# openzklib/openzl

Measured on AMD Instinct MI355X. Metric: MSM points/sec (BLS12-381 G1), higher is better.
Workload: dtype u32; 1 GPU; bls12_381_g1_msm_2^24_per_gpu; points_per_gpu=16777216, curve=BLS12-381 G1, scalars=uniform < r (255 bit), window_bits=20, windows=13, precomputed_table=none (the fixed-key table mode is reported separately as msm_fixed_key), parallelism=single

## Files before the change

### openzl_amd/csrc/zl_msm.hip

```cpp
#include <stdlib.h>
#include <string.h>
#include <stdio.h>
#include <algorithm>
#include <chrono>
#include <condition_variable>
#include <mutex>
#include <thread>
#include <vector>
#include "zl_ctx.h"
#include "zl_pool.h"
#include "zl_quad.h"

#ifndef ZL_G
#error "compile with -DZL_G=<group config>"
#endif
#include "zl_msm_job.h"
#include "zl_msm_bases.h"
ZL_MSM_ACCUMULATE_KERNELS(extern, ZL_G)
ZL_MSM_TAIL_KERNELS(extern, ZL_G)

template <class G>
static int msm_run_t(zl_ctx* ctx, const zl_bases& bs, size_t first, const void* d_scalars, size_t n, uint64_t* out_partial) {
    using X = XYZZ<typename G::F>;
    X total = X::inf();
// ... 67 lines not shown
    for (size_t i = 0; i < count; i++) any_empty = any_empty || specs[i].n == 0;
    if (any_empty || count == 1) {
        for (size_t i = 0; i < count; i++) {
            if (recorded) { while (recorded->load(std::memory_order_acquire) >= 0 && recorded->load(std::memory_order_acquire) <= (int)i) std::this_thread::yield(); if (recorded->load() < 0) return ZL_EHIP; }
            if (specs[i].wait) ZL_HIP(ctx, hipEventSynchronize(specs[i].wait));
            int rc = msm_run_t<G>(ctx, *specs[i].bs, specs[i].first, specs[i].d_scalars, specs[i].n, out_partials + i * ZL_PARTIAL_WORDS);
            if (rc) return rc;
            if (on_done) (*on_done)(i);
        }
        return ZL_OK;
    }
    int rc;
    struct Busy {
        std::atomic<int>& f;
        bool mine;
        explicit Busy(std::atomic<int>& x) : f(x), mine(x.exchange(1, std::memory_order_acq_rel) == 0) {}
        ~Busy() { if (mine) f.store(0, std::memory_order_release); }
    } busy(ctx->pipeline_busy);
    if (!busy.mine) return ZL_EINVAL;
    if (!ctx->stream_sort) {
        int prio_lo = 0, prio_hi = 0;
        (void)hipDeviceGetStreamPriorityRange(&prio_lo, &prio_hi);
        ZL_HIP(ctx, hipStreamCreateWithPriority(&ctx->stream_sort, hipStreamNonBlocking, prio_hi));
        for (auto& t : ctx->stream_tail) ZL_HIP(ctx, hipStreamCreateWithPriority(&t, hipStreamNonBlocking, prio_hi));
    }
    std::vector<MsmJob<G>> jobs(count);
    size_t t5 = 0, t6 = 0;
    uint32_t max_sets = 0;
    bool one_key = true;
    for (size_t i = 1; i < count; i++) one_key = one_key && specs[i].bs == specs[0].bs && specs[i].first == specs[0].first && specs[i].n == specs[0].n;
    uint64_t biggest = 0;
    for (size_t i = 0; i < count; i++) biggest = std::max<uint64_t>(biggest, (uint64_t)specs[i].n);
    const bool side = biggest <= ((uint64_t)1 << zl_tune("ZL_TUNE_SIDE_BY_SIDE_LOG", 20));
    const size_t NS = side ? std::min<size_t>(count, (size_t)std::min(4, std::max(1, zl_tune("ZL_TUNE_SIDE_LANES", 4)))) : 3;
    for (size_t i = 0; i < count; i++) {
        if ((rc = jobs[i].plan(ctx, *specs[i].bs, specs[i].first, specs[i].d_scalars, specs[i].n, (one_key && !side) ? 18 : MsmJob<G>::phi_slot_of((int)(i % NS))))) return rc;
        if (one_key && !side && i > 0) jobs[i].phi_owner = false;
        size_t a5, a6;
        jobs[i].sort_tmp_sizes(a5, a6);
        t5 = std::max(t5, a5);
        t6 = std::max(t6, a6);
        max_sets = std::max<uint32_t>(max_sets, jobs[i].SETS * jobs[i].roots_per_set);
    }
    hipStream_t* const lanes = ctx->stream_lane;
    if (side) {
        for (size_t k = 0; k < 4; k++)
            if (!lanes[k]) ZL_HIP(ctx, hipStreamCreateWithFlags(&lanes[k], hipStreamNonBlocking));
    }
    void* dummy;
    if (!side && t5 && (rc = zl_scratch_get(ctx, 5, t5, &dummy))) return rc;
    if (!side && t6 && (rc = zl_scratch_get(ctx, 6, t6, &dummy))) return rc;
    for (int pass = 0; pass < 2; pass++) {
        for (size_t i = 0; i < count; i++) {
            if ((rc = jobs[i].alloc(ctx, (int)(i % NS), side))) return rc;
            if (one_key && !side && i > 0 && jobs[i].glv && !jobs[i].phi_cached) jobs[i].d_phi = jobs[0].d_phi;
        }
    }
    const size_t per = sizeof(X) * (max_sets + 1) + 16;
    if (ctx->pinned_cap < per * count) {
        const size_t want = std::max(per * count, (sizeof(X) * 320 + 16) * (size_t)24);
        if (ctx->pinned) (void)hipHostFree(ctx->pinned);
        ctx->pinned = nullptr;
        ctx->pinned_cap = 0;
        ZL_HIP(ctx, hipHostMalloc(&ctx->pinned, want, hipHostMallocDefault));
        ctx->pinned_cap = want;
    }
    for (size_t i = 0; i < count; i++) {
        unsigned char* base = reinterpret_cast<unsigned char*>(ctx->pinned) + per * i;
        jobs[i].set_host_buffer(reinterpret_cast<X*>(base));
    }
// ... 450 lines not shown
```

### openzl_amd/csrc/zl_msm_job.h

```cpp
#pragma once
#include <chrono>
#include <stdlib.h>
#include <string.h>
#include <stdio.h>
#include <algorithm>
#include <vector>
#include "zl_ctx.h"
#include "zl_pool.h"
#include "zl_msm_sort.h"
#include "zl_msm_endo.h"
#include "zl_msm_accumulate.h"
#include "zl_msm_reduce.h"

static int zl_pick_window(size_t n, int sc_bits, bool wide16 = false ) {
    const double per_bucket = (double)zl_tune("ZL_TUNE_BUCKET_COST_X10", sc_bits > 200 ? 45 : 52) / 10.0;
    double best = 1e300;
    int best_c = 2;
    for (int c = 2; c <= 20; c++) {
        int W = (sc_bits + 1 + c - 1) / c;
        if (c > 16 && (((uint64_t)W << (c - 1)) >> 15) > 255) continue;
        const bool lds_sort = c < 16 || (c == 16 && !wide16);
        double cost = (double)n * W * (lds_sort ? 1.10 : 1.0) + per_bucket * W * (double)(1u << (c - 1));
        if (cost < best) { best = cost; best_c = c; }
    }
// ... 9 lines not shown
}
static int zl_pick_window_quarter(size_t n_points) {
    if (n_points < 2) return 0;
    int lg = 63 - __builtin_clzll((unsigned long long)n_points);
    if ((double)n_points >= 1.4142 * (double)((size_t)1 << lg)) lg++;
    static const signed char best[9] = {9, 0, 11, 12, 13, 13, 13, 13, 14};
    return lg >= 10 && lg <= 18 ? best[lg - 10] : 0;
}

static int zl_pick_window_precomp(size_t n, int sc_bits) {
    if (n < (size_t)700000) return 16;
    if (n < ((size_t)1 << 21)) return 20;
    double best = 1e300;
    int best_c = 16;
    for (int c = 20; c <= 23; c++) {
        int W = (sc_bits + 1 + c - 1) / c;
        double cost = (double)n * W + 6.0 * (double)(1u << (c - 1));
        if (cost < best) { best = cost; best_c = c; }
    }
    return best_c;
}

template <class G>
struct MsmJob {
    using F = typename G::F;
    using X = XYZZ<F>;
    bool pre = false;
    int c = 0, W = 0;
    int spread_t = -1;
    bool wide = false;
    bool glv = false;
    bool phi_cached = false;
    bool phi_owner = false;
    int sc_bits = 0, phi_slot = -1, endo_k = 1;
    int slotA = 5, slotB = 6;
    size_t n_real = 0;
    uint32_t* d_vs = nullptr;
    const Affine<F>* d_phi = nullptr;
    uint32_t H = 0, SETS = 0, NB = 0, ZL_CHUNK = 0, nchunks = 0, scan_blocks = 0, max_big = 0, max_giant = 0, Gn = 0, big_span = ZL_BIG_SPAN;
    uint32_t red_g0 = 0, red_lg0 = 0, red_blocks = 0, red_levels = 0;
    uint32_t roots_per_set = 0;
    uint64_t maxE = 0;
    size_t n = 0, first = 0;
    const zl_bases* bsp = nullptr;
    uint32_t *d_counts = nullptr, *d_offsets = nullptr, *d_cursor = nullptr, *d_entries = nullptr, *d_block_sums = nullptr, *d_big_list = nullptr,
             *d_big_count = nullptr, *d_ones_count = nullptr, *d_giant_count = nullptr, *d_giant_list = nullptr, *d_ones_list = nullptr,
             *d_bigsg_items = nullptr, *d_bad_scalar = nullptr;
    unsigned long long* d_bigsg_head = nullptr;
    X *d_buckets = nullptr, *d_partials = nullptr, *d_segs = nullptr, *d_stage1 = nullptr, *d_sets = nullptr, *d_ones_parts = nullptr, *d_giant_tmp = nullptr;
    const Affine<F>* d_bases = nullptr;
    const uint8_t* d_inf = nullptr;
    const uint32_t* sc = nullptr;
    X* hw = nullptr;
    uint32_t* hE = nullptr;
    std::vector<X> hw_own;
    void set_host_buffer(X* buf) {
        hw = buf;
        hE = reinterpret_cast<uint32_t*>(buf + (size_t)SETS * roots_per_set + 1);
    }

    int plan(zl_ctx* ctx, const zl_bases& bs, size_t first_, const void* d_scalars, size_t n_, int phi_slot_ = -1) {
        static const bool no_glv = getenv("ZL_NO_GLV") != nullptr;
        bool try_glv = false;
        static const size_t glv_max = (size_t)1 << zl_tune("ZL_TUNE_GLV_MAX_LOG", 19);
        if constexpr (G::GLV) try_glv = phi_slot_ >= 0 && bs.precomp_c == 0 && !no_glv && n_ >= 1 && n_ <= glv_max && (uint64_t)n_ * G::ENDO_K < (1ull << 31);
        if constexpr (G::GLV && G::ENDO_K == 2) {
// ... 212 lines not shown
        }
        const int glv_i = glv ? 1 : 0;
        (void)hipFuncSetAttribute(reinterpret_cast<const void*>(&k_msm_hist_lds), hipFuncAttributeMaxDynamicSharedMemorySize, 128 * 1024);
        (void)hipFuncSetAttribute(reinterpret_cast<const void*>(&k_msm_scatter_range), hipFuncAttributeMaxDynamicSharedMemorySize, 128 * 1024);
        if (wide) rc = sort_wide(ctx, st, sc_eff, inf_eff, bad_eff, nblk, glv_i);
        else if (c <= 16) rc = sort_lds(ctx, st, sc_eff, inf_eff, bad_eff, nblk, glv_i);
        else rc = sort_atomics(ctx, st, nblk);
        if (rc) return rc;
        ZL_HIP(ctx, hipGetLastError());
        return ZL_OK;
    }
    int sort_wide(zl_ctx* ctx, hipStream_t st, const uint32_t* sc_eff, const uint8_t* inf_eff, uint32_t* bad_eff, uint32_t nblk, int glv_i) {
        const zl_bases& bs = *bsp;
        int rc;
        uint32_t nslices = 64;
        const uint32_t max_slices = (uint32_t)((n + 4095) / 4096);
        if (nslices > max_slices) nslices = max_slices;
        const uint32_t per_slice = (uint32_t)((n + nslices - 1) / nslices);
        const uint32_t P = Gn * W * nslices;
        const uint32_t pscan_blocks = (P + SCAN_BLOCK * SCAN_ITEMS - 1) / (SCAN_BLOCK * SCAN_ITEMS);
        const size_t b_lo = (((size_t)n * W * 2 + 255) / 256) * 256, b_hi = (((size_t)n * W + 255) / 256) * 256;
        const size_t b_plo = b_lo, b_pidx = (((size_t)n * W * 4 + 255) / 256) * 256;
        const size_t b_pc = (((size_t)(2 * P + pscan_blocks + 8) * 4 + 255) / 256) * 256;
        void* pd;
        if ((rc = zl_scratch_get(ctx, slotA, b_lo + b_hi + b_plo + b_pidx + b_pc + 256, &pd))) return rc;
        unsigned char* q = (unsigned char*)pd;
        uint16_t* d_lo16 = (uint16_t*)q; q += b_lo;
        uint8_t* d_hi8 = (uint8_t*)q; q += b_hi;
        uint16_t* d_part_lo = (uint16_t*)q; q += b_plo;
        uint32_t* d_part_idx = (uint32_t*)q; q += b_pidx;
        uint32_t* d_pcounts = (uint32_t*)q;
        uint32_t* d_poff = d_pcounts + P;
        uint32_t* d_pblock = d_poff + P + 1;
        hipLaunchKernelGGL(k_msm_recode_wide, dim3(nblk), dim3(256), 0, st, sc_eff, (uint32_t)n, c, W, pre ? 0u : (H >> 15), spread_t, glv_i, d_lo16, d_hi8, d_ones_list, d_ones_count, inf_eff, sc_bits, bad_eff);
        hipLaunchKernelGGL(k_msm_part_hist, dim3(nslices, W), dim3(256), 0, st, d_hi8, (uint32_t)n, (uint32_t)W, Gn, per_slice, nslices, d_pcounts);
        hipLaunchKernelGGL(k_scan_block_sums, dim3(pscan_blocks), dim3(SCAN_BLOCK), 0, st, d_pcounts, P, d_pblock);
        hipLaunchKernelGGL(k_scan_top, dim3(1), dim3(1024), 0, st, d_pblock, pscan_blocks, d_poff + P, (const uint32_t*)nullptr);
        hipLaunchKernelGGL(k_scan_apply, dim3(pscan_blocks), dim3(SCAN_BLOCK), 0, st, d_pcounts, P, d_pblock, d_poff, d_pcounts);
        hipLaunchKernelGGL(k_msm_part_scatter_st, dim3(nslices, W), dim3(256), 0, st, d_lo16, d_hi8, (uint32_t)n, (uint32_t)W, Gn, per_slice, nslices, d_poff,
                           pre ? (uint32_t)bs.n : 0u, pre ? (uint32_t)first : 0u, d_part_lo, d_part_idx);
        const uint32_t gstride = (uint32_t)W * nslices;
        const uint32_t SG = Gn * 128;
        uint32_t fsl = 16;
        while (fsl * Gn < 2048 && fsl < 128) fsl *= 2;
        const uint32_t P2 = SG * fsl;
        const uint32_t p2scan_blocks = (P2 + SCAN_BLOCK * SCAN_ITEMS - 1) / (SCAN_BLOCK * SCAN_ITEMS);
        void* pd2;
        const size_t b2_lo = b_plo, b2_idx = b_pidx, b2_c = (((size_t)(2 * (size_t)P2 + p2scan_blocks + 8) * 4 + 255) / 256) * 256;
        if ((rc = zl_scratch_get(ctx, slotB, b2_lo + b2_idx + b2_c + 256, &pd2))) return rc;
        unsigned char* q2 = (unsigned char*)pd2;
        uint16_t* d_lo2 = (uint16_t*)q2; q2 += b2_lo;
        uint32_t* d_idx2 = (uint32_t*)q2; q2 += b2_idx;
        uint32_t* d_c2 = (uint32_t*)q2;
        uint32_t* d_off2 = d_c2 + P2;
        uint32_t* d_blk2 = d_off2 + P2 + 1;
        hipLaunchKernelGGL(k_msm_sub_hist, dim3(fsl, Gn), dim3(256), 0, st, d_part_lo, d_poff, Gn, gstride, d_poff + P, fsl, d_c2);
        hipLaunchKernelGGL(k_scan_block_sums, dim3(p2scan_blocks), dim3(SCAN_BLOCK), 0, st, d_c2, P2, d_blk2);
        hipLaunchKernelGGL(k_scan_top, dim3(1), dim3(1024), 0, st, d_blk2, p2scan_blocks, d_off2 + P2, (const uint32_t*)nullptr);
        hipLaunchKernelGGL(k_scan_apply, dim3(p2scan_blocks), dim3(SCAN_BLOCK), 0, st, d_c2, P2, d_blk2, d_off2, d_c2);
        hipLaunchKernelGGL(k_msm_sub_scatter_st, dim3(fsl, Gn), dim3(256), 0, st, d_part_lo, d_part_idx, d_poff, Gn, gstride, d_poff + P, fsl, d_off2, d_lo2,
                           d_idx2);
        hipLaunchKernelGGL(k_msm_fine_hist, dim3(SG), dim3(256), 0, st, d_lo2, d_off2, SG, fsl, d_off2 + P2, d_counts);
        hipLaunchKernelGGL(k_scan_block_sums, dim3(scan_blocks), dim3(SCAN_BLOCK), 0, st, d_counts, NB, d_block_sums);
        hipLaunchKernelGGL(k_scan_top, dim3(1), dim3(1024), 0, st, d_block_sums, scan_blocks, d_offsets + NB, (const uint32_t*)d_bad_scalar);
        hipLaunchKernelGGL(k_scan_apply, dim3(scan_blocks), dim3(SCAN_BLOCK), 0, st, d_counts, NB, d_block_sums, d_offsets, d_cursor);
        uint32_t cap = (uint32_t)std::min<uint64_t>(36 * 1024, std::max<uint64_t>(4096, (maxE / SG) * 22 / 10));
        cap = (uint32_t)std::max(1024, zl_tune("ZL_TUNE_FS_CAP", (int)cap));
        (void)hipFuncSetAttribute(reinterpret_cast<const void*>(&k_msm_fine_sort), hipFuncAttributeMaxDynamicSharedMemorySize, 160 * 1024);
        hipLaunchKernelGGL(k_msm_fine_sort, dim3(SG), dim3(zl_tune("ZL_TUNE_FS", 1024)), (size_t)(256 + cap) * 4, st, d_lo2, d_idx2, d_off2, SG, fsl, d_off2 + P2, d_offsets, cap,
                           d_entries, d_bigsg_head, d_bigsg_items);
        (void)hipFuncSetAttribute(reinterpret_cast<const void*>(&k_msm_fine_sort_big), hipFuncAttributeMaxDynamicSharedMemorySize, ZL_BT * 4);
        hipLaunchKernelGGL(k_msm_fine_sort_big, dim3(512), dim3(1024), (size_t)ZL_BT * 4, st, d_lo2, d_idx2, d_off2, SG, fsl, d_off2 + P2, d_bigsg_head,
                           d_bigsg_items, d_cursor, d_entries);
        return ZL_OK;
    }
    int sort_lds(zl_ctx* ctx, hipStream_t st, const uint32_t* sc_eff, const uint8_t* inf_eff, uint32_t* bad_eff, uint32_t nblk, int glv_i) {
        int rc;
        uint32_t nslices = (256 + W - 1) / W;
        const uint32_t max_slices = (uint32_t)((n + 4095) / 4096);
        if (nslices > max_slices) nslices = max_slices;
        if (nslices < 1) nslices = 1;
        const uint32_t per_slice = (uint32_t)((n + nslices - 1) / nslices);
        void* pd;
        if ((rc = zl_scratch_get(ctx, slotA, (size_t)n * W * 2 + (size_t)nslices * NB * 4 + 256, &pd))) return rc;
        uint16_t* d_digits = (uint16_t*)pd;
        uint32_t* d_slice_counts = (uint32_t*)((unsigned char*)pd + (((size_t)n * W * 2 + 255) / 256) * 256);
        hipLaunchKernelGGL(k_msm_recode, dim3(nblk), dim3(256), 0, st, sc_eff, (uint32_t)n, c, W, spread_t, glv_i, d_digits, d_ones_list, d_ones_count, inf_eff, sc_bits, bad_eff);
        hipLaunchKernelGGL(k_msm_hist_lds, dim3(nslices, W), dim3(1024), (size_t)H * 4, st, d_digits, (uint32_t)n, H, per_slice, NB, d_slice_counts);
        if (NB <= 14336 && nslices <= 64) {
            hipLaunchKernelGGL(k_msm_prefix_small, dim3(1), dim3(1024), ((size_t)NB + NB / 16 + 16) * 4, st, d_slice_counts, NB, nslices, d_offsets, d_cursor, (const uint32_t*)d_bad_scalar);
        } else {
        hipLaunchKernelGGL(k_msm_slice_prefix, dim3((NB + 255) / 256), dim3(256), 0, st, d_slice_counts, NB, nslices, d_counts);
        hipLaunchKernelGGL(k_scan_block_sums, dim3(scan_blocks), dim3(SCAN_BLOCK), 0, st, d_counts, NB, d_block_sums);
        hipLaunchKernelGGL(k_scan_top, dim3(1), dim3(1024), 0, st, d_block_sums, scan_blocks, d_offsets + NB, (const uint32_t*)d_bad_scalar);
        hipLaunchKernelGGL(k_scan_apply, dim3(scan_blocks), dim3(SCAN_BLOCK), 0, st, d_counts, NB, d_block_sums, d_offsets, d_cursor);
        }
        uint32_t ranges = 1;
        while (ranges * W < 256 && (H / (ranges * 2)) >= 64) ranges *= 2;
// ... 138 lines not shown
```

### openzl_amd/csrc/zl_msm_sort.h

```cpp
#pragma once
#include "zl_msm_common.h"

#define ZL_PT 4096
#define ZL_BT 16384
#define SCAN_ITEMS 16
#define SCAN_BLOCK 256

__global__ void __launch_bounds__(64) k_msm_zero_words(uint32_t* __restrict__ p, uint32_t n);
template <int MODE>
__global__ void __launch_bounds__(256) k_msm_digits(const uint32_t* __restrict__ scalars, uint32_t n, int c, int W,
                                                    uint32_t* __restrict__ counters, uint32_t* __restrict__ entries,
                                                    uint32_t* __restrict__ ones_list, uint32_t* __restrict__ ones_count, const uint8_t* __restrict__ inf,
                                                    int sc_bits, uint32_t* __restrict__ bad);
__global__ void __launch_bounds__(256) k_msm_recode(const uint32_t* __restrict__ scalars, uint32_t n, int c, int W, int spread_t, int glv, uint16_t* __restrict__ digits,
                                                             uint32_t* __restrict__ ones_list, uint32_t* __restrict__ ones_count, const uint8_t* __restrict__ inf,
                                                             int sc_bits, uint32_t* __restrict__ bad);
__global__ void __launch_bounds__(1024) k_msm_hist_lds(const uint16_t* __restrict__ digits, uint32_t n, uint32_t H, uint32_t per_slice, uint32_t NB,
                                                        uint32_t* __restrict__ counts);
__global__ void __launch_bounds__(256) k_msm_slice_prefix(uint32_t* __restrict__ counts, uint32_t NB, uint32_t nslices, uint32_t* __restrict__ tot);
__global__ void __launch_bounds__(1024) k_msm_scatter_range(const uint16_t* __restrict__ digits, uint32_t n, uint32_t H, uint32_t RB,
                                                                     const uint32_t* __restrict__ offsets, uint32_t* __restrict__ entries,
                                                                     const uint32_t* __restrict__ slice_prefix, uint32_t NB, uint32_t nslices, uint32_t per_slice,
                                                                     uint32_t parts, uint32_t W);
__global__ void __launch_bounds__(256) k_msm_recode_wide(const uint32_t* __restrict__ scalars, uint32_t n, int c, int W, uint32_t gw, int spread_t, int glv,
// ... 2 lines not shown
                                                                  int sc_bits, uint32_t* __restrict__ bad);
__global__ void __launch_bounds__(256) k_msm_part_hist(const uint8_t* __restrict__ hi8, uint32_t n, uint32_t W, uint32_t G, uint32_t per_slice,
                                                                uint32_t nslices, uint32_t* __restrict__ counts);
__global__ void __launch_bounds__(256) k_msm_sub_hist(const uint16_t* __restrict__ part_lo, const uint32_t* __restrict__ part_off, uint32_t G,
                                                               uint32_t stride, const uint32_t* __restrict__ total, uint32_t fslices,
                                                               uint32_t* __restrict__ counts);
__global__ void __launch_bounds__(256) k_msm_part_scatter_st(const uint16_t* __restrict__ lo16, const uint8_t* __restrict__ hi8, uint32_t n, uint32_t W,
                                                                      uint32_t G, uint32_t per_slice, uint32_t nslices, const uint32_t* __restrict__ part_off,
                                                                      uint32_t table_stride, uint32_t first, uint16_t* __restrict__ out_lo,
                                                                      uint32_t* __restrict__ out_idx);
__global__ void __launch_bounds__(256) k_msm_sub_scatter_st(const uint16_t* __restrict__ part_lo, const uint32_t* __restrict__ part_idx,
                                                                     const uint32_t* __restrict__ part_off, uint32_t G, uint32_t stride,
                                                                     const uint32_t* __restrict__ total, uint32_t fslices, const uint32_t* __restrict__ sub_off,
                                                                     uint16_t* __restrict__ out_lo, uint32_t* __restrict__ out_idx);
__global__ void __launch_bounds__(256) k_msm_fine_hist(const uint16_t* __restrict__ lo2, const uint32_t* __restrict__ sub_off, uint32_t SG,
                                                                uint32_t fslices, const uint32_t* __restrict__ total, uint32_t* __restrict__ counts);
__global__ void __launch_bounds__(1024) k_msm_fine_sort(const uint16_t* __restrict__ lo2, const uint32_t* __restrict__ idx2,
                                                                const uint32_t* __restrict__ sub_off, uint32_t SG, uint32_t fslices,
                                                                const uint32_t* __restrict__ total, const uint32_t* __restrict__ offsets, uint32_t cap,
                                                                uint32_t* __restrict__ entries, unsigned long long* __restrict__ big_head,
                                                                uint32_t* __restrict__ big_items);
__global__ void __launch_bounds__(1024) k_msm_fine_sort_big(const uint16_t* __restrict__ lo2, const uint32_t* __restrict__ idx2,
                                                                    const uint32_t* __restrict__ sub_off, uint32_t SG, uint32_t fslices,
                                                                    const uint32_t* __restrict__ total, const unsigned long long* __restrict__ big_head,
                                                                    const uint32_t* __restrict__ big_items, uint32_t* __restrict__ cursor,
                                                                    uint32_t* __restrict__ entries);
__global__ void __launch_bounds__(SCAN_BLOCK) k_scan_block_sums(const uint32_t* __restrict__ in, uint32_t count, uint32_t* __restrict__ block_sums);
__global__ void __launch_bounds__(1024) k_scan_top(uint32_t* __restrict__ block_sums, uint32_t nblocks, uint32_t* __restrict__ total_out,
                                                          const uint32_t* __restrict__ flag_in = nullptr );
__global__ void __launch_bounds__(1024) k_msm_prefix_small(uint32_t* __restrict__ counts, uint32_t NB, uint32_t nslices, uint32_t* __restrict__ offsets,
                                                                  uint32_t* __restrict__ cursor, const uint32_t* __restrict__ flag_in);
__global__ void __launch_bounds__(SCAN_BLOCK) k_scan_apply(const uint32_t* __restrict__ in, uint32_t count, const uint32_t* __restrict__ block_sums,
                                                           uint32_t* __restrict__ out, uint32_t* __restrict__ out2);
```

### openzl_amd/csrc/zl_msm_sort.hip

```cpp
#include "zl_msm_sort.h"



__device__ __forceinline__ bool zl_take_one(const uint32_t* s, uint32_t i, uint32_t* __restrict__ ones_list, uint32_t* __restrict__ ones_count) {
    const bool one = s[0] == 1u && (s[1] | s[2] | s[3] | s[4] | s[5] | s[6] | s[7]) == 0u;
    const uint64_t m = __ballot(one);
    if (m == 0) return false;
    const uint32_t lane = threadIdx.x & 63u;
    uint32_t base = 0;
    if (lane == (uint32_t)__ffsll((long long)m) - 1u) base = atomicAdd(ones_count, (uint32_t)__popcll(m));
    base = __shfl(base, __ffsll((long long)m) - 1);
    if (one) ones_list[base + __popcll(m & ((1ull << lane) - 1ull))] = i;
    return one;
}

__device__ __forceinline__ uint32_t zl_take_sign(uint32_t& top_word, int glv) {
    if (!glv) return 0u;
    const uint32_t sg = top_word >> 31;
    top_word &= 0x7FFFFFFFu;
    return sg;
}
__global__ void __launch_bounds__(64) k_msm_zero_words(uint32_t* __restrict__ p, uint32_t n) {
    if (threadIdx.x < n) p[threadIdx.x] = 0u;
}
// ... 188 lines not shown
    uint4 lo = sp[0], hi = sp[1];
    if (live) zl_flag_wide_scalar(hi.w, sc_bits, bad);
    if (!live || (inf && inf[i])) lo = hi = make_uint4(0, 0, 0, 0);
    uint32_t s[8] = {lo.x, lo.y, lo.z, lo.w, hi.x, hi.y, hi.z, hi.w};
    if (zl_take_one(s, i, ones_list, ones_count)) s[0] = 0;
    if (!live) return;
    const uint32_t sg = zl_take_sign(s[7], glv);
    const uint32_t H = 1u << (c - 1);
    uint32_t carry = 0;
    for (int w = 0; w < W; w++) {
        const int pos = w * c;
        const int word = pos >> 5, sh = pos & 31;
        uint64_t v = 0;
#pragma unroll
        for (int k = 0; k < 8; k++) {
            if (k == word) v |= s[k];
            if (k == word + 1) v |= (uint64_t)s[k] << 32;
        }
        uint32_t d = ((uint32_t)(v >> sh) & ((1u << c) - 1)) + carry;
        uint32_t neg = 0;
        carry = 0;
        if (d > H) { d = 2 * H - d; neg = 1; carry = 1; }
        uint32_t b = d - 1;
        if (spread_t >= 0 && w == W - 1) b |= (i & ((1u << (c - 1 - spread_t)) - 1u)) << spread_t;
        lo16[(size_t)w * n + i] = (uint16_t)((b & 0x7FFFu) | ((neg ^ sg) << 15));
        hi8[(size_t)w * n + i] = d == 0 ? (uint8_t)0xFF : (uint8_t)((uint32_t)w * gw + (b >> 15));
    }
}
__global__ void __launch_bounds__(256) k_msm_part_hist(const uint8_t* __restrict__ hi8, uint32_t n, uint32_t W, uint32_t G, uint32_t per_slice,
                                                                uint32_t nslices, uint32_t* __restrict__ counts) {
    ZL_SIDE_PRIO();
    __shared__ uint32_t hist[256];
    const uint32_t slice = blockIdx.x, w = blockIdx.y;
    hist[threadIdx.x] = 0;
    __syncthreads();
    const uint32_t lo = slice * per_slice, hi = min(n, lo + per_slice);
    const uint8_t* hw = hi8 + (size_t)w * n;
    const bool al = ((((size_t)w * n) | lo) & 15) == 0;
    const uint32_t body1 = al ? lo + ((hi - lo) & ~15u) : lo;
    const uint4* hv = reinterpret_cast<const uint4*>(hw);
    for (uint32_t i16 = lo / 16 + threadIdx.x; i16 < body1 / 16; i16 += blockDim.x) {
        const uint4 v = hv[i16];
        const uint32_t words[4] = {v.x, v.y, v.z, v.w};
#pragma unroll
        for (int k = 0; k < 16; k++) {
            const uint32_t g = (words[k >> 2] >> ((k & 3) * 8)) & 0xFFu;
            if (g != 0xFFu) atomicAdd(&hist[g], 1u);
        }
    }
    for (uint32_t i = body1 + threadIdx.x; i < hi; i += blockDim.x) {
        const uint32_t g = hw[i];
        if (g != 0xFFu) atomicAdd(&hist[g], 1u);
    }
    __syncthreads();
    if (threadIdx.x < G) counts[((size_t)threadIdx.x * W + w) * nslices + slice] = hist[threadIdx.x];
}
__device__ __forceinline__ void zl_group_range(const uint32_t* __restrict__ part_off, uint32_t g, uint32_t G, uint32_t stride, uint32_t E, uint32_t& s,
                                               uint32_t& e) {
    s = part_off[(size_t)g * stride];
    e = (g + 1 < G) ? part_off[(size_t)(g + 1) * stride] : E;
}
__global__ void __launch_bounds__(256) k_msm_sub_hist(const uint16_t* __restrict__ part_lo, const uint32_t* __restrict__ part_off, uint32_t G,
                                                               uint32_t stride, const uint32_t* __restrict__ total, uint32_t fslices,
                                                               uint32_t* __restrict__ counts) {
    ZL_SIDE_PRIO();
    __shared__ uint32_t hist[128];
    const uint32_t slice = blockIdx.x, g = blockIdx.y;
    if (threadIdx.x < 128) hist[threadIdx.x] = 0;
    __syncthreads();
    uint32_t s, e;
    zl_group_range(part_off, g, G, stride, *total, s, e);
    const uint32_t per = (e - s + fslices - 1) / fslices;
    const uint32_t lo = min(e, s + slice * per), hi = min(e, lo + per);
    const uint32_t body0 = min(hi, (lo + 7u) & ~7u), body1 = max(body0, hi & ~7u);
    for (uint32_t j = lo + threadIdx.x; j < body0; j += blockDim.x) atomicAdd(&hist[(part_lo[j] >> 8) & 127u], 1u);
    const uint4* dv = reinterpret_cast<const uint4*>(part_lo);
    for (uint32_t j8 = body0 / 8 + threadIdx.x; j8 < body1 / 8; j8 += blockDim.x) {
        const uint4 v = dv[j8];
        const uint32_t words[4] = {v.x, v.y, v.z, v.w};
#pragma unroll
        for (int k = 0; k < 8; k++) atomicAdd(&hist[((words[k >> 1] >> ((k & 1) * 16)) >> 8) & 127u], 1u);
    }
    for (uint32_t j = body1 + threadIdx.x; j < hi; j += blockDim.x) atomicAdd(&hist[(part_lo[j] >> 8) & 127u], 1u);
    __syncthreads();
    if (threadIdx.x < 128) counts[((size_t)g * 128 + threadIdx.x) * fslices + slice] = hist[threadIdx.x];
}
struct PartStage {
    uint32_t gcur[256];
    uint32_t hist[256];
    uint32_t start[257];
    uint32_t idx[ZL_PT];
    uint16_t code[ZL_PT];
};
__device__ __forceinline__ void zl_part_scan(PartStage& st) {
    __shared__ uint32_t wsum[4];
    const uint32_t v = st.hist[threadIdx.x];
    uint32_t x = v;
#pragma unroll
    for (int off = 1; off < 64; off <<= 1) {
        const uint32_t y = __shfl_up(x, off);
        if ((threadIdx.x & 63) >= (uint32_t)off) x += y;
    }
    if ((threadIdx.x & 63) == 63) wsum[threadIdx.x >> 6] = x;
    __syncthreads();
    uint32_t base = 0;
    for (uint32_t w = 0; w < (threadIdx.x >> 6); w++) base += wsum[w];
    st.start[threadIdx.x] = base + x - v;
    if (threadIdx.x == 255) st.start[256] = base + x;
    __syncthreads();
}
template <class BinFn, class OutFn>
__device__ __forceinline__ void zl_part_flush(PartStage& st, uint32_t cnt, uint16_t* __restrict__ out_lo, uint32_t* __restrict__ out_idx, BinFn binfn, OutFn outfn) {
    for (uint32_t j = threadIdx.x; j < cnt; j += 256) {
        const uint32_t code = st.code[j];
        const uint32_t b = binfn(code);
        const uint32_t dest = st.gcur[b] + (j - st.start[b]);
        out_lo[dest] = (uint16_t)outfn(code);
        out_idx[dest] = st.idx[j];
// ... 95 lines not shown
            const uint32_t cw[8] = {c0.x, c0.y, c0.z, c0.w, c1.x, c1.y, c1.z, c1.w};
            const uint32_t iw[16] = {i0.x, i0.y, i0.z, i0.w, i1.x, i1.y, i1.z, i1.w, i2.x, i2.y, i2.z, i2.w, i3.x, i3.y, i3.z, i3.w};
#pragma unroll
            for (int k = 0; k < EPT; k++) {
                code[k] = (cw[k >> 1] >> ((k & 1) * 16)) & 0xFFFFu;
                idx[k] = iw[k];
                ok[k] = true;
            }
        } else {
#pragma unroll
            for (int k = 0; k < EPT; k++) {
                ok[k] = j0 + k >= lo && j0 + k < hi;
                code[k] = ok[k] ? part_lo[j0 + k] : 0u;
                idx[k] = ok[k] ? part_idx[j0 + k] : 0u;
            }
        }
#pragma unroll
        for (int k = 0; k < EPT; k++) rank[k] = ok[k] ? atomicAdd(&st.hist[(code[k] >> 8) & 127u], 1u) : 0u;
        __syncthreads();
        zl_part_scan(st);
#pragma unroll
        for (int k = 0; k < EPT; k++) {
            if (ok[k]) {
                const uint32_t pos = st.start[(code[k] >> 8) & 127u] + rank[k];
                st.code[pos] = (uint16_t)code[k];
                st.idx[pos] = idx[k];
            }
        }
        __syncthreads();
        zl_part_flush(st, st.start[256], out_lo, out_idx, [](uint32_t c) { return (c >> 8) & 127u; },
                      [](uint32_t c) { return (c & 0xFFu) | (c & 0x8000u); });
    }
}
__global__ void __launch_bounds__(256) k_msm_fine_hist(const uint16_t* __restrict__ lo2, const uint32_t* __restrict__ sub_off, uint32_t SG,
                                                                uint32_t fslices, const uint32_t* __restrict__ total, uint32_t* __restrict__ counts) {
    ZL_SIDE_PRIO();
    __shared__ uint32_t hist[256];
    const uint32_t sg = blockIdx.x;
    hist[threadIdx.x] = 0;
    __syncthreads();
    const uint32_t s = sub_off[(size_t)sg * fslices], e = (sg + 1 < SG) ? sub_off[(size_t)(sg + 1) * fslices] : *total;
    const uint32_t body0 = min(e, (s + 7u) & ~7u), body1 = max(body0, e & ~7u);
    for (uint32_t j = s + threadIdx.x; j < body0; j += blockDim.x) atomicAdd(&hist[lo2[j] & 0xFFu], 1u);
    const uint4* dv = reinterpret_cast<const uint4*>(lo2);
    for (uint32_t j8 = body0 / 8 + threadIdx.x; j8 < body1 / 8; j8 += blockDim.x) {
        const uint4 v = dv[j8];
        const uint32_t words[4] = {v.x, v.y, v.z, v.w};
#pragma unroll
        for (int k = 0; k < 8; k++) atomicAdd(&hist[(words[k >> 1] >> ((k & 1) * 16)) & 0xFFu], 1u);
    }
    for (uint32_t j = body1 + threadIdx.x; j < e; j += blockDim.x) atomicAdd(&hist[lo2[j] & 0xFFu], 1u);
    __syncthreads();
    counts[(size_t)sg * 256 + threadIdx.x] = hist[threadIdx.x];
}
__global__ void __launch_bounds__(1024) k_msm_fine_sort(const uint16_t* __restrict__ lo2, const uint32_t* __restrict__ idx2,
                                                                const uint32_t* __restrict__ sub_off, uint32_t SG, uint32_t fslices,
                                                                const uint32_t* __restrict__ total, const uint32_t* __restrict__ offsets, uint32_t cap,
                                                                uint32_t* __restrict__ entries, unsigned long long* __restrict__ big_head,
                                                                uint32_t* __restrict__ big_items) {
    ZL_SIDE_PRIO();
    extern __shared__ __attribute__((aligned(16))) unsigned char smem[];
    uint32_t* cur = reinterpret_cast<uint32_t*>(smem);
    uint32_t* stage = cur + 256;
    const uint32_t sg = blockIdx.x;
    const uint32_t s = sub_off[(size_t)sg * fslices], e = (sg + 1 < SG) ? sub_off[(size_t)(sg + 1) * fslices] : *total;
    const uint32_t base = offsets[(size_t)sg * 256];
    const uint32_t len = e - s;
    if (len > cap) {
        if (threadIdx.x == 0) {
            const uint32_t tiles = (len + ZL_BT - 1) / ZL_BT;
            const unsigned long long old = atomicAdd(big_head, (1ull << 32) | tiles);
            const uint32_t item = (uint32_t)(old >> 32);
            big_items[2 * item] = sg;
            big_items[2 * item + 1] = (uint32_t)old;
        }
        return;
    }
    for (uint32_t b = threadIdx.x; b < 256; b += blockDim.x) cur[b] = offsets[(size_t)sg * 256 + b] - base;
    __syncthreads();
    for (uint32_t j = s + threadIdx.x; j < e; j += blockDim.x) {
        const uint32_t code = lo2[j];
        const uint32_t pos = atomicAdd(&cur[code & 0xFFu], 1u);
        stage[pos] = idx2[j] | ((code >> 15) << 31);
    }
    __syncthreads();
    for (uint32_t k = threadIdx.x; k < len; k += blockDim.x) entries[base + k] = stage[k];
// ... 158 lines not shown
    for (uint32_t b = threadIdx.x; b < NB; b += 1024) {
        const uint32_t o = tot[b + (b >> 4)];
        offsets[b] = o;
        cursor[b] = o;
    }
    if (threadIdx.x == 1023) {
        offsets[NB] = sh[1023];
        if (flag_in) offsets[NB + 1] = *flag_in;
    }
}
__global__ void __launch_bounds__(SCAN_BLOCK) k_scan_apply(const uint32_t* __restrict__ in, uint32_t count, const uint32_t* __restrict__ block_sums,
                                                           uint32_t* __restrict__ out, uint32_t* __restrict__ out2) {
    ZL_SIDE_PRIO();
    __shared__ uint32_t sh[SCAN_BLOCK];
    uint32_t base = blockIdx.x * SCAN_BLOCK * SCAN_ITEMS + threadIdx.x * SCAN_ITEMS;
    uint32_t v[SCAN_ITEMS];
    uint32_t s = 0;
    for (int k = 0; k < SCAN_ITEMS; k++) { v[k] = (base + k < count) ? in[base + k] : 0; s += v[k]; }
    sh[threadIdx.x] = s;
    __syncthreads();
    for (int off = 1; off < SCAN_BLOCK; off <<= 1) {
        uint32_t t = threadIdx.x >= off ? sh[threadIdx.x - off] : 0;
        __syncthreads();
        sh[threadIdx.x] += t;
        __syncthreads();
    }
    uint32_t run = block_sums[blockIdx.x] + sh[threadIdx.x] - s;
    for (int k = 0; k < SCAN_ITEMS; k++) {
        if (base + k < count) { out[base + k] = run; out2[base + k] = run; }
        run += v[k];
    }
}

template __global__ void k_msm_digits<0>(const uint32_t*, uint32_t, int, int, uint32_t*, uint32_t*, uint32_t*, uint32_t*, const uint8_t*, int, uint32_t*);
template __global__ void k_msm_digits<1>(const uint32_t*, uint32_t, int, int, uint32_t*, uint32_t*, uint32_t*, uint32_t*, const uint8_t*, int, uint32_t*);
```

Baseline: 459.7 million points/s.

## Run the bucket sort pipeline with single-wavefront blocks and add a fourth pipeline set

```diff
diff --git a/openzl_amd/csrc/zl_msm.hip b/openzl_amd/csrc/zl_msm.hip
--- a/openzl_amd/csrc/zl_msm.hip
+++ b/openzl_amd/csrc/zl_msm.hip
@@ -123,10 +123,12 @@
     uint64_t biggest = 0;
     for (size_t i = 0; i < count; i++) biggest = std::max<uint64_t>(biggest, (uint64_t)specs[i].n);
     const bool side = biggest <= ((uint64_t)1 << zl_tune("ZL_TUNE_SIDE_BY_SIDE_LOG", 20));
-    const size_t NS = side ? std::min<size_t>(count, (size_t)std::min(4, std::max(1, zl_tune("ZL_TUNE_SIDE_LANES", 4)))) : 3;
+    const size_t NS = side ? std::min<size_t>(count, (size_t)std::min(4, std::max(1, zl_tune("ZL_TUNE_SIDE_LANES", 4))))
+                           : (size_t)std::min(4, std::max(3, zl_tune("ZL_TUNE_PIPE_SETS", 4)));
     for (size_t i = 0; i < count; i++) {
         if ((rc = jobs[i].plan(ctx, *specs[i].bs, specs[i].first, specs[i].d_scalars, specs[i].n, (one_key && !side) ? 18 : MsmJob<G>::phi_slot_of((int)(i % NS))))) return rc;
         if (one_key && !side && i > 0) jobs[i].phi_owner = false;
+        jobs[i].one_wave = !side && zl_tune("ZL_TUNE_SORT_ONE_WAVE", 1);
         size_t a5, a6;
         jobs[i].sort_tmp_sizes(a5, a6);
         t5 = std::max(t5, a5);
diff --git a/openzl_amd/csrc/zl_msm_job.h b/openzl_amd/csrc/zl_msm_job.h
--- a/openzl_amd/csrc/zl_msm_job.h
+++ b/openzl_amd/csrc/zl_msm_job.h
@@ -65,6 +65,7 @@
     bool glv = false;
     bool phi_cached = false;
     bool phi_owner = false;
+    bool one_wave = false;
     int sc_bits = 0, phi_slot = -1, endo_k = 1;
     int slotA = 5, slotB = 6;
     size_t n_real = 0;
@@ -343,13 +344,27 @@
         uint32_t* d_pcounts = (uint32_t*)q;
         uint32_t* d_poff = d_pcounts + P;
         uint32_t* d_pblock = d_poff + P + 1;
-        hipLaunchKernelGGL(k_msm_recode_wide, dim3(nblk), dim3(256), 0, st, sc_eff, (uint32_t)n, c, W, pre ? 0u : (H >> 15), spread_t, glv_i, d_lo16, d_hi8, d_ones_list, d_ones_count, inf_eff, sc_bits, bad_eff);
-        hipLaunchKernelGGL(k_msm_part_hist, dim3(nslices, W), dim3(256), 0, st, d_hi8, (uint32_t)n, (uint32_t)W, Gn, per_slice, nslices, d_pcounts);
-        hipLaunchKernelGGL(k_scan_block_sums, dim3(pscan_blocks), dim3(SCAN_BLOCK), 0, st, d_pcounts, P, d_pblock);
-        hipLaunchKernelGGL(k_scan_top, dim3(1), dim3(1024), 0, st, d_pblock, pscan_blocks, d_poff + P, (const uint32_t*)nullptr);
-        hipLaunchKernelGGL(k_scan_apply, dim3(pscan_blocks), dim3(SCAN_BLOCK), 0, st, d_pcounts, P, d_pblock, d_poff, d_pcounts);
-        hipLaunchKernelGGL(k_msm_part_scatter_st, dim3(nslices, W), dim3(256), 0, st, d_lo16, d_hi8, (uint32_t)n, (uint32_t)W, Gn, per_slice, nslices, d_poff,
-                           pre ? (uint32_t)bs.n : 0u, pre ? (uint32_t)first : 0u, d_part_lo, d_part_idx);
+        const uint32_t lanes = one_wave ? 64u : 256u;
+        auto scan = [&](const uint32_t* cnt, uint32_t count, uint32_t blocks, uint32_t* blk, uint32_t* tot, const uint32_t* flag, uint32_t* out, uint32_t* out2) {
+            if (one_wave) {
+                hipLaunchKernelGGL(k_scan_block_sums_w, dim3(blocks), dim3(64), 0, st, cnt, count, blk);
+                hipLaunchKernelGGL(k_scan_top_w, dim3(1), dim3(64), 0, st, blk, blocks, tot, flag);
+                hipLaunchKernelGGL(k_scan_apply_w, dim3(blocks), dim3(64), 0, st, cnt, count, blk, out, out2);
+            } else {
+                hipLaunchKernelGGL(k_scan_block_sums, dim3(blocks), dim3(SCAN_BLOCK), 0, st, cnt, count, blk);
+                hipLaunchKernelGGL(k_scan_top, dim3(1), dim3(1024), 0, st, blk, blocks, tot, flag);
+                hipLaunchKernelGGL(k_scan_apply, dim3(blocks), dim3(SCAN_BLOCK), 0, st, cnt, count, blk, out, out2);
+            }
+        };
+        hipLaunchKernelGGL(k_msm_recode_wide, dim3((uint32_t)((n + lanes - 1) / lanes)), dim3(lanes), 0, st, sc_eff, (uint32_t)n, c, W, pre ? 0u : (H >> 15), spread_t, glv_i, d_lo16, d_hi8, d_ones_list, d_ones_count, inf_eff, sc_bits, bad_eff);
+        hipLaunchKernelGGL(k_msm_part_hist, dim3(nslices, W), dim3(lanes), 0, st, d_hi8, (uint32_t)n, (uint32_t)W, Gn, per_slice, nslices, d_pcounts);
+        scan(d_pcounts, P, pscan_blocks, d_pblock, d_poff + P, nullptr, d_poff, d_pcounts);
+        if (one_wave)
+            hipLaunchKernelGGL(k_msm_part_scatter_w, dim3(nslices, W), dim3(64), 0, st, d_lo16, d_hi8, (uint32_t)n, (uint32_t)W, Gn, per_slice, nslices, d_poff,
+                               pre ? (uint32_t)bs.n : 0u, pre ? (uint32_t)first : 0u, d_part_lo, d_part_idx);
+        else
+            hipLaunchKernelGGL(k_msm_part_scatter_st, dim3(nslices, W), dim3(256), 0, st, d_lo16, d_hi8, (uint32_t)n, (uint32_t)W, Gn, per_slice, nslices, d_poff,
+                               pre ? (uint32_t)bs.n : 0u, pre ? (uint32_t)first : 0u, d_part_lo, d_part_idx);
         const uint32_t gstride = (uint32_t)W * nslices;
         const uint32_t SG = Gn * 128;
         uint32_t fsl = 16;
@@ -365,16 +380,15 @@
         uint32_t* d_c2 = (uint32_t*)q2;
         uint32_t* d_off2 = d_c2 + P2;
         uint32_t* d_blk2 = d_off2 + P2 + 1;
-        hipLaunchKernelGGL(k_msm_sub_hist, dim3(fsl, Gn), dim3(256), 0, st, d_part_lo, d_poff, Gn, gstride, d_poff + P, fsl, d_c2);
-        hipLaunchKernelGGL(k_scan_block_sums, dim3(p2scan_blocks), dim3(SCAN_BLOCK), 0, st, d_c2, P2, d_blk2);
-        hipLaunchKernelGGL(k_scan_top, dim3(1), dim3(1024), 0, st, d_blk2, p2scan_blocks, d_off2 + P2, (const uint32_t*)nullptr);
-        hipLaunchKernelGGL(k_scan_apply, dim3(p2scan_blocks), dim3(SCAN_BLOCK), 0, st, d_c2, P2, d_blk2, d_off2, d_c2);
-        hipLaunchKernelGGL(k_msm_sub_scatter_st, dim3(fsl, Gn), dim3(256), 0, st, d_part_lo, d_part_idx, d_poff, Gn, gstride, d_poff + P, fsl, d_off2, d_lo2,
-                           d_idx2);
-        hipLaunchKernelGGL(k_msm_fine_hist, dim3(SG), dim3(256), 0, st, d_lo2, d_off2, SG, fsl, d_off2 + P2, d_counts);
-        hipLaunchKernelGGL(k_scan_block_sums, dim3(scan_blocks), dim3(SCAN_BLOCK), 0, st, d_counts, NB, d_block_sums);
-        hipLaunchKernelGGL(k_scan_top, dim3(1), dim3(1024), 0, st, d_block_sums, scan_blocks, d_offsets + NB, (const uint32_t*)d_bad_scalar);
-        hipLaunchKernelGGL(k_scan_apply, dim3(scan_blocks), dim3(SCAN_BLOCK), 0, st, d_counts, NB, d_block_sums, d_offsets, d_cursor);
+        hipLaunchKernelGGL(k_msm_sub_hist, dim3(fsl, Gn), dim3(lanes), 0, st, d_part_lo, d_poff, Gn, gstride, d_poff + P, fsl, d_c2);
+        scan(d_c2, P2, p2scan_blocks, d_blk2, d_off2 + P2, nullptr, d_off2, d_c2);
+        if (one_wave)
+            hipLaunchKernelGGL(k_msm_sub_scatter_w, dim3(fsl, Gn), dim3(64), 0, st, d_part_lo, d_part_idx, d_poff, Gn, gstride, d_poff + P, fsl, d_off2, d_lo2, d_idx2);
+        else
+            hipLaunchKernelGGL(k_msm_sub_scatter_st, dim3(fsl, Gn), dim3(256), 0, st, d_part_lo, d_part_idx, d_poff, Gn, gstride, d_poff + P, fsl, d_off2, d_lo2,
+                               d_idx2);
+        hipLaunchKernelGGL(k_msm_fine_hist, dim3(SG), dim3(lanes), 0, st, d_lo2, d_off2, SG, fsl, d_off2 + P2, d_counts);
+        scan(d_counts, NB, scan_blocks, d_block_sums, d_offsets + NB, d_bad_scalar, d_offsets, d_cursor);
         uint32_t cap = (uint32_t)std::min<uint64_t>(36 * 1024, std::max<uint64_t>(4096, (maxE / SG) * 22 / 10));
         cap = (uint32_t)std::max(1024, zl_tune("ZL_TUNE_FS_CAP", (int)cap));
         (void)hipFuncSetAttribute(reinterpret_cast<const void*>(&k_msm_fine_sort), hipFuncAttributeMaxDynamicSharedMemorySize, 160 * 1024);
diff --git a/openzl_amd/csrc/zl_msm_sort.h b/openzl_amd/csrc/zl_msm_sort.h
--- a/openzl_amd/csrc/zl_msm_sort.h
+++ b/openzl_amd/csrc/zl_msm_sort.h
@@ -58,3 +58,16 @@
                                                                   uint32_t* __restrict__ cursor, const uint32_t* __restrict__ flag_in);
 __global__ void __launch_bounds__(SCAN_BLOCK) k_scan_apply(const uint32_t* __restrict__ in, uint32_t count, const uint32_t* __restrict__ block_sums,
                                                            uint32_t* __restrict__ out, uint32_t* __restrict__ out2);
+__global__ void __launch_bounds__(64) k_msm_part_scatter_w(const uint16_t* __restrict__ lo16, const uint8_t* __restrict__ hi8, uint32_t n, uint32_t W,
+                                                            uint32_t G, uint32_t per_slice, uint32_t nslices, const uint32_t* __restrict__ part_off,
+                                                            uint32_t table_stride, uint32_t first, uint16_t* __restrict__ out_lo,
+                                                            uint32_t* __restrict__ out_idx);
+__global__ void __launch_bounds__(64) k_msm_sub_scatter_w(const uint16_t* __restrict__ part_lo, const uint32_t* __restrict__ part_idx,
+                                                           const uint32_t* __restrict__ part_off, uint32_t G, uint32_t stride,
+                                                           const uint32_t* __restrict__ total, uint32_t fslices, const uint32_t* __restrict__ sub_off,
+                                                           uint16_t* __restrict__ out_lo, uint32_t* __restrict__ out_idx);
+__global__ void __launch_bounds__(64) k_scan_block_sums_w(const uint32_t* __restrict__ in, uint32_t count, uint32_t* __restrict__ block_sums);
+__global__ void __launch_bounds__(64) k_scan_top_w(uint32_t* __restrict__ block_sums, uint32_t nblocks, uint32_t* __restrict__ total_out,
+                                                    const uint32_t* __restrict__ flag_in);
+__global__ void __launch_bounds__(64) k_scan_apply_w(const uint32_t* __restrict__ in, uint32_t count, const uint32_t* __restrict__ block_sums,
+                                                      uint32_t* __restrict__ out, uint32_t* __restrict__ out2);
diff --git a/openzl_amd/csrc/zl_msm_sort.hip b/openzl_amd/csrc/zl_msm_sort.hip
--- a/openzl_amd/csrc/zl_msm_sort.hip
+++ b/openzl_amd/csrc/zl_msm_sort.hip
@@ -244,7 +244,7 @@
     ZL_SIDE_PRIO();
     __shared__ uint32_t hist[256];
     const uint32_t slice = blockIdx.x, w = blockIdx.y;
-    hist[threadIdx.x] = 0;
+    for (uint32_t b = threadIdx.x; b < 256; b += blockDim.x) hist[b] = 0;
     __syncthreads();
     const uint32_t lo = slice * per_slice, hi = min(n, lo + per_slice);
     const uint8_t* hw = hi8 + (size_t)w * n;
@@ -265,7 +265,7 @@
         if (g != 0xFFu) atomicAdd(&hist[g], 1u);
     }
     __syncthreads();
-    if (threadIdx.x < G) counts[((size_t)threadIdx.x * W + w) * nslices + slice] = hist[threadIdx.x];
+    for (uint32_t b = threadIdx.x; b < G; b += blockDim.x) counts[((size_t)b * W + w) * nslices + slice] = hist[b];
 }
 __device__ __forceinline__ void zl_group_range(const uint32_t* __restrict__ part_off, uint32_t g, uint32_t G, uint32_t stride, uint32_t E, uint32_t& s,
                                                uint32_t& e) {
@@ -278,7 +278,7 @@
     ZL_SIDE_PRIO();
     __shared__ uint32_t hist[128];
     const uint32_t slice = blockIdx.x, g = blockIdx.y;
-    if (threadIdx.x < 128) hist[threadIdx.x] = 0;
+    for (uint32_t b = threadIdx.x; b < 128; b += blockDim.x) hist[b] = 0;
     __syncthreads();
     uint32_t s, e;
     zl_group_range(part_off, g, G, stride, *total, s, e);
@@ -295,7 +295,7 @@
     }
     for (uint32_t j = body1 + threadIdx.x; j < hi; j += blockDim.x) atomicAdd(&hist[(part_lo[j] >> 8) & 127u], 1u);
     __syncthreads();
-    if (threadIdx.x < 128) counts[((size_t)g * 128 + threadIdx.x) * fslices + slice] = hist[threadIdx.x];
+    for (uint32_t b = threadIdx.x; b < 128; b += blockDim.x) counts[((size_t)g * 128 + b) * fslices + slice] = hist[b];
 }
 struct PartStage {
     uint32_t gcur[256];
@@ -457,12 +457,204 @@
                       [](uint32_t c) { return (c & 0xFFu) | (c & 0x8000u); });
     }
 }
+__device__ __forceinline__ void zl_part_scan_w(PartStage& st) {
+    const uint32_t l = threadIdx.x;
+    const uint32_t v0 = st.hist[4 * l], v1 = st.hist[4 * l + 1], v2 = st.hist[4 * l + 2], v3 = st.hist[4 * l + 3];
+    const uint32_t v = v0 + v1 + v2 + v3;
+    uint32_t x = v;
+#pragma unroll
+    for (int off = 1; off < 64; off <<= 1) {
+        const uint32_t y = __shfl_up(x, off);
+        if (l >= (uint32_t)off) x += y;
+    }
+    const uint32_t b0 = x - v;
+    st.start[4 * l] = st.hist[4 * l] = b0;
+    st.start[4 * l + 1] = st.hist[4 * l + 1] = b0 + v0;
+    st.start[4 * l + 2] = st.hist[4 * l + 2] = b0 + v0 + v1;
+    st.start[4 * l + 3] = st.hist[4 * l + 3] = b0 + v0 + v1 + v2;
+    if (l == 63) st.start[256] = x;
+    __syncthreads();
+}
+__device__ __forceinline__ void zl_part_next_w(PartStage& st) {
+    for (uint32_t b = threadIdx.x; b < 256; b += 64) {
+        st.gcur[b] += st.start[b + 1] - st.start[b];
+        st.hist[b] = 0;
+    }
+    __syncthreads();
+}
+__global__ void __launch_bounds__(64) k_msm_part_scatter_w(const uint16_t* __restrict__ lo16, const uint8_t* __restrict__ hi8, uint32_t n, uint32_t W,
+                                                            uint32_t G, uint32_t per_slice, uint32_t nslices, const uint32_t* __restrict__ part_off,
+                                                            uint32_t table_stride, uint32_t first, uint16_t* __restrict__ out_lo,
+                                                            uint32_t* __restrict__ out_idx) {
+    ZL_SIDE_PRIO();
+    __shared__ PartStage st;
+    __shared__ uint8_t grp[ZL_PT];
+    const uint32_t slice = blockIdx.x, w = blockIdx.y, l = threadIdx.x;
+    for (uint32_t b = l; b < 256; b += 64) {
+        st.gcur[b] = b < G ? part_off[((size_t)b * W + w) * nslices + slice] : 0u;
+        st.hist[b] = 0;
+    }
+    __syncthreads();
+    const uint32_t lo = slice * per_slice, hi = min(n, lo + per_slice);
+    const uint8_t* hw = hi8 + (size_t)w * n;
+    const uint16_t* lw = lo16 + (size_t)w * n;
+    const uint32_t add = w * table_stride + first;
+    const bool al = ((((size_t)w * n) | lo) & 15) == 0;
+    constexpr int EPT = 16;
+    for (uint32_t t0 = lo; t0 < hi; t0 += ZL_PT) {
+        for (uint32_t j0 = t0 + l * EPT; j0 < min(hi, t0 + ZL_PT); j0 += 64 * EPT) {
+            uint32_t g[EPT];
+            if (al && j0 + EPT <= hi) {
+                const uint4 v = *reinterpret_cast<const uint4*>(hw + j0);
+                const uint32_t words[4] = {v.x, v.y, v.z, v.w};
+#pragma unroll
+                for (int k = 0; k < EPT; k++) g[k] = (words[k >> 2] >> ((k & 3) * 8)) & 0xFFu;
+            } else {
+#pragma unroll
+                for (int k = 0; k < EPT; k++) g[k] = j0 + k < hi ? hw[j0 + k] : 0xFFu;
+            }
+#pragma unroll
+            for (int k = 0; k < EPT; k++)
+                if (g[k] != 0xFFu) atomicAdd(&st.hist[g[k]], 1u);
+        }
+        __syncthreads();
+        zl_part_scan_w(st);
+        for (uint32_t j0 = t0 + l * EPT; j0 < min(hi, t0 + ZL_PT); j0 += 64 * EPT) {
+            uint32_t g[EPT], code[EPT];
+            if (al && j0 + EPT <= hi) {
+                const uint4 v = *reinterpret_cast<const uint4*>(hw + j0);
+                const uint4 l0 = *reinterpret_cast<const uint4*>(lw + j0), l1 = *reinterpret_cast<const uint4*>(lw + j0 + 8);
+                const uint32_t words[4] = {v.x, v.y, v.z, v.w};
+                const uint32_t lws[8] = {l0.x, l0.y, l0.z, l0.w, l1.x, l1.y, l1.z, l1.w};
+#pragma unroll
+                for (int k = 0; k < EPT; k++) {
+                    g[k] = (words[k >> 2] >> ((k & 3) * 8)) & 0xFFu;
+                    code[k] = (lws[k >> 1] >> ((k & 1) * 16)) & 0xFFFFu;
+                }
+            } else {
+#pragma unroll
+                for (int k = 0; k < EPT; k++) {
+                    const bool ok = j0 + k < hi;
+                    g[k] = ok ? hw[j0 + k] : 0xFFu;
+                    code[k] = ok ? lw[j0 + k] : 0u;
+                }
+            }
+#pragma unroll
+            for (int k = 0; k < EPT; k++) {
+                if (g[k] != 0xFFu) {
+                    const uint32_t pos = atomicAdd(&st.hist[g[k]], 1u);
+                    st.code[pos] = (uint16_t)code[k];
+                    st.idx[pos] = add + j0 + k;
+                    grp[pos] = (uint8_t)g[k];
+                }
+            }
+        }
+        __syncthreads();
+        const uint32_t cnt = st.start[256];
+        for (uint32_t j = l; j < cnt; j += 64) {
+            const uint32_t b = grp[j];
+            const uint32_t dest = st.gcur[b] + (j - st.start[b]);
+            out_lo[dest] = st.code[j];
+            out_idx[dest] = st.idx[j];
+        }
+        __syncthreads();
+        zl_part_next_w(st);
+    }
+}
+__global__ void __launch_bounds__(64) k_msm_sub_scatter_w(const uint16_t* __restrict__ part_lo, const uint32_t* __restrict__ part_idx,
+                                                           const uint32_t* __restrict__ part_off, uint32_t G, uint32_t stride,
+                                                           const uint32_t* __restrict__ total, uint32_t fslices, const uint32_t* __restrict__ sub_off,
+                                                           uint16_t* __restrict__ out_lo, uint32_t* __restrict__ out_idx) {
+    ZL_SIDE_PRIO();
+    __shared__ PartStage st;
+    const uint32_t slice = blockIdx.x, g = blockIdx.y, l = threadIdx.x;
+    for (uint32_t b = l; b < 256; b += 64) {
+        st.gcur[b] = b < 128 ? sub_off[((size_t)g * 128 + b) * fslices + slice] : 0u;
+        st.hist[b] = 0;
+    }
+    __syncthreads();
+    uint32_t s, e;
+    zl_group_range(part_off, g, G, stride, *total, s, e);
+    const uint32_t per = (e - s + fslices - 1) / fslices;
+    const uint32_t lo = min(e, s + slice * per), hi = min(e, lo + per);
+    constexpr int EPT = 16;
+    const uint32_t a0 = lo & ~7u;
+    for (uint32_t t0 = a0; t0 < hi; t0 += ZL_PT) {
+        for (uint32_t j0 = t0 + l * EPT; j0 < min(hi, t0 + ZL_PT); j0 += 64 * EPT) {
+            uint32_t code[EPT];
+            bool ok[EPT];
+            if (j0 >= lo && j0 + EPT <= hi) {
+                const uint4 c0 = *reinterpret_cast<const uint4*>(part_lo + j0), c1 = *reinterpret_cast<const uint4*>(part_lo + j0 + 8);
+                const uint32_t cw[8] = {c0.x, c0.y, c0.z, c0.w, c1.x, c1.y, c1.z, c1.w};
+#pragma unroll
+                for (int k = 0; k < EPT; k++) {
+                    code[k] = (cw[k >> 1] >> ((k & 1) * 16)) & 0xFFFFu;
+                    ok[k] = true;
+                }
+            } else {
+#pragma unroll
+                for (int k = 0; k < EPT; k++) {
+                    ok[k] = j0 + k >= lo && j0 + k < hi;
+                    code[k] = ok[k] ? part_lo[j0 + k] : 0u;
+                }
+            }
+#pragma unroll
+            for (int k = 0; k < EPT; k++)
+                if (ok[k]) atomicAdd(&st.hist[(code[k] >> 8) & 127u], 1u);
+        }
+        __syncthreads();
+        zl_part_scan_w(st);
+        for (uint32_t j0 = t0 + l * EPT; j0 < min(hi, t0 + ZL_PT); j0 += 64 * EPT) {
+            uint32_t code[EPT], idx[EPT];
+            bool ok[EPT];
+            if (j0 >= lo && j0 + EPT <= hi) {
+                const uint4 c0 = *reinterpret_cast<const uint4*>(part_lo + j0), c1 = *reinterpret_cast<const uint4*>(part_lo + j0 + 8);
+                const uint4* iv = reinterpret_cast<const uint4*>(part_idx + j0);
+                const uint4 i0 = iv[0], i1 = iv[1], i2 = iv[2], i3 = iv[3];
+                const uint32_t cw[8] = {c0.x, c0.y, c0.z, c0.w, c1.x, c1.y, c1.z, c1.w};
+                const uint32_t iw[16] = {i0.x, i0.y, i0.z, i0.w, i1.x, i1.y, i1.z, i1.w, i2.x, i2.y, i2.z, i2.w, i3.x, i3.y, i3.z, i3.w};
+#pragma unroll
+                for (int k = 0; k < EPT; k++) {
+                    code[k] = (cw[k >> 1] >> ((k & 1) * 16)) & 0xFFFFu;
+                    idx[k] = iw[k];
+                    ok[k] = true;
+                }
+            } else {
+#pragma unroll
+                for (int k = 0; k < EPT; k++) {
+                    ok[k] = j0 + k >= lo && j0 + k < hi;
+                    code[k] = ok[k] ? part_lo[j0 + k] : 0u;
+                    idx[k] = ok[k] ? part_idx[j0 + k] : 0u;
+                }
+            }
+#pragma unroll
+            for (int k = 0; k < EPT; k++) {
+                if (ok[k]) {
+                    const uint32_t pos = atomicAdd(&st.hist[(code[k] >> 8) & 127u], 1u);
+                    st.code[pos] = (uint16_t)code[k];
+                    st.idx[pos] = idx[k];
+                }
+            }
+        }
+        __syncthreads();
+        const uint32_t cnt = st.start[256];
+        for (uint32_t j = l; j < cnt; j += 64) {
+            const uint32_t c = st.code[j];
+            const uint32_t b = (c >> 8) & 127u;
+            const uint32_t dest = st.gcur[b] + (j - st.start[b]);
+            out_lo[dest] = (uint16_t)((c & 0xFFu) | (c & 0x8000u));
+            out_idx[dest] = st.idx[j];
+        }
+        __syncthreads();
+        zl_part_next_w(st);
+    }
+}
 __global__ void __launch_bounds__(256) k_msm_fine_hist(const uint16_t* __restrict__ lo2, const uint32_t* __restrict__ sub_off, uint32_t SG,
                                                                 uint32_t fslices, const uint32_t* __restrict__ total, uint32_t* __restrict__ counts) {
     ZL_SIDE_PRIO();
     __shared__ uint32_t hist[256];
     const uint32_t sg = blockIdx.x;
-    hist[threadIdx.x] = 0;
+    for (uint32_t b = threadIdx.x; b < 256; b += blockDim.x) hist[b] = 0;
     __syncthreads();
     const uint32_t s = sub_off[(size_t)sg * fslices], e = (sg + 1 < SG) ? sub_off[(size_t)(sg + 1) * fslices] : *total;
     const uint32_t body0 = min(e, (s + 7u) & ~7u), body1 = max(body0, e & ~7u);
@@ -476,7 +668,7 @@
     }
     for (uint32_t j = body1 + threadIdx.x; j < e; j += blockDim.x) atomicAdd(&hist[lo2[j] & 0xFFu], 1u);
     __syncthreads();
-    counts[(size_t)sg * 256 + threadIdx.x] = hist[threadIdx.x];
+    for (uint32_t b = threadIdx.x; b < 256; b += blockDim.x) counts[(size_t)sg * 256 + b] = hist[b];
 }
 __global__ void __launch_bounds__(1024) k_msm_fine_sort(const uint16_t* __restrict__ lo2, const uint32_t* __restrict__ idx2,
                                                                 const uint32_t* __restrict__ sub_off, uint32_t SG, uint32_t fslices,
@@ -701,5 +893,58 @@
     }
 }
 
+__device__ __forceinline__ uint32_t zl_wave_incl_scan(uint32_t x) {
+#pragma unroll
+    for (int off = 1; off < 64; off <<= 1) {
+        const uint32_t y = __shfl_up(x, off);
+        if (threadIdx.x >= (uint32_t)off) x += y;
+    }
+    return x;
+}
+__global__ void __launch_bounds__(64) k_scan_block_sums_w(const uint32_t* __restrict__ in, uint32_t count, uint32_t* __restrict__ block_sums) {
+    ZL_SIDE_PRIO();
+    uint32_t s = 0;
+    for (uint32_t r = 0; r < SCAN_BLOCK / 64; r++) {
+        const uint32_t base = blockIdx.x * SCAN_BLOCK * SCAN_ITEMS + (r * 64 + threadIdx.x) * SCAN_ITEMS;
+        for (int k = 0; k < SCAN_ITEMS; k++) if (base + k < count) s += in[base + k];
+    }
+    s = zl_wave_incl_scan(s);
+    if (threadIdx.x == 63) block_sums[blockIdx.x] = s;
+}
+__global__ void __launch_bounds__(64) k_scan_top_w(uint32_t* __restrict__ block_sums, uint32_t nblocks, uint32_t* __restrict__ total_out,
+                                                    const uint32_t* __restrict__ flag_in) {
+    ZL_SIDE_PRIO();
+    uint32_t carry = 0;
+    for (uint32_t base = 0; base < nblocks; base += 64) {
+        const uint32_t idx = base + threadIdx.x;
+        const uint32_t v = idx < nblocks ? block_sums[idx] : 0;
+        const uint32_t x = zl_wave_incl_scan(v);
+        if (idx < nblocks) block_sums[idx] = carry + x - v;
+        carry += __shfl(x, 63);
+    }
+    if (threadIdx.x == 0) {
+        *total_out = carry;
+        if (flag_in) total_out[1] = *flag_in;
+    }
+}
+__global__ void __launch_bounds__(64) k_scan_apply_w(const uint32_t* __restrict__ in, uint32_t count, const uint32_t* __restrict__ block_sums,
+                                                      uint32_t* __restrict__ out, uint32_t* __restrict__ out2) {
+    ZL_SIDE_PRIO();
+    uint32_t carry = block_sums[blockIdx.x];
+    for (uint32_t r = 0; r < SCAN_BLOCK / 64; r++) {
+        const uint32_t base = blockIdx.x * SCAN_BLOCK * SCAN_ITEMS + (r * 64 + threadIdx.x) * SCAN_ITEMS;
+        uint32_t v[SCAN_ITEMS];
+        uint32_t s = 0;
+        for (int k = 0; k < SCAN_ITEMS; k++) { v[k] = (base + k < count) ? in[base + k] : 0; s += v[k]; }
+        const uint32_t x = zl_wave_incl_scan(s);
+        uint32_t run = carry + x - s;
+        for (int k = 0; k < SCAN_ITEMS; k++) {
+            if (base + k < count) { out[base + k] = run; out2[base + k] = run; }
+            run += v[k];
+        }
+        carry += __shfl(x, 63);
+    }
+}
+
 template __global__ void k_msm_digits<0>(const uint32_t*, uint32_t, int, int, uint32_t*, uint32_t*, uint32_t*, uint32_t*, const uint8_t*, int, uint32_t*);
 template __global__ void k_msm_digits<1>(const uint32_t*, uint32_t, int, int, uint32_t*, uint32_t*, uint32_t*, uint32_t*, const uint8_t*, int, uint32_t*);
```

New measurement: 469.2 million points/s, median of 6. 1.02x the previous value.
